# stijnherfst/Tyrant

Measured on AMD Instinct MI355X. Metric: Mrays/s at 1080p 8spp, higher is better.
Workload: dtype f32

## Files before the change

### tyrant_amd/csrc/hip/traverse.hpp

```cpp
#pragma once

#include <type_traits>

#include <hip/hip_runtime.h>

#include "vecmath.hpp"

namespace tyr {

constexpr uint32_t kRefLeaf = 0x80000000u;
constexpr uint32_t kRefDone = 0xFFFFFFFFu;
constexpr uint32_t kRefPop = 0xFFFFFFFEu;
constexpr int kStackSize = 64;
constexpr uint32_t kMaxLeafPrims = 31;
constexpr uint32_t kMaxPrimOffset = 1u << 26;
constexpr uint32_t kStagedNodes = 64;
constexpr uint32_t kQuadOrderShift = 25;
constexpr uint32_t kQuadIndexMask = (1u << kQuadOrderShift) - 1u;

struct DevScene {
	const float4* quads;
	uint32_t quadRootRef;
	uint32_t nQuads;
	uint32_t nStaged;
// ... 177 lines not shown
		lds = (lds_column_t)ldsColumn;
		spillRef = refs;
		spillT = ts;
	}
	__device__ __forceinline__ void reset() {
		n = 0;
		overflow = false;
	}
	__device__ __forceinline__ void lds_put(int d, uint32_t r, float t) {
		if constexpr (WITH_T)
			lds[d * kBlockThreads] = make_uint2(r, __float_as_uint(t));
		else
			lds[d * kBlockThreads] = r;
	}
	__device__ __forceinline__ void lds_get(int d, uint32_t& r, float& t) {
		if constexpr (WITH_T) {
			const uint2 e = lds[d * kBlockThreads];
			r = e.x;
			t = __uint_as_float(e.y);
		} else {
			r = lds[d * kBlockThreads];
			t = -__builtin_inff();
		}
	}
	__device__ __forceinline__ void push(uint32_t r, float t) {
		if (LDS_DEPTH > 0 && n < LDS_DEPTH) {
			lds_put(n, r, t);
			++n;
		} else if (n < kStackSize) {
			spillRef[n - LDS_DEPTH] = r;
			if (WITH_T)
				spillT[n - LDS_DEPTH] = t;
			++n;
		} else {
			overflow = true;
		}
	}
	__device__ __forceinline__ bool pop(uint32_t& r, float& t) {
		if (n == 0)
			return false;
		if (LDS_DEPTH > 0 && __builtin_amdgcn_ballot_w64(n > LDS_DEPTH) == 0ull) {
			--n;
			lds_get(n, r, t);
			return true;
		}
		--n;
		if (LDS_DEPTH > 0 && n < LDS_DEPTH) {
			lds_get(n, r, t);
		} else {
			r = spillRef[n - LDS_DEPTH];
			t = WITH_T ? spillT[n - LDS_DEPTH] : -__builtin_inff();
		}
		return true;
	}
	__device__ __forceinline__ void push3(unsigned long long ma, uint32_t ra, float ta, unsigned long long mb, uint32_t rb, float tb, unsigned long long mc, uint32_t rc, float tc) {
		if (LDS_DEPTH >= 3 && __builtin_amdgcn_ballot_w64(n > LDS_DEPTH - 3) == 0ull) {
			if (__builtin_amdgcn_inverse_ballot_w64(ma)) {
				lds_put(n, ra, ta);
				++n;
			}
			if (__builtin_amdgcn_inverse_ballot_w64(mb)) {
				lds_put(n, rb, tb);
				++n;
			}
			if (__builtin_amdgcn_inverse_ballot_w64(mc)) {
				lds_put(n, rc, tc);
				++n;
			}
			return;
		}
		if (__builtin_amdgcn_inverse_ballot_w64(ma))
			push(ra, ta);
		if (__builtin_amdgcn_inverse_ballot_w64(mb))
			push(rb, tb);
		if (__builtin_amdgcn_inverse_ballot_w64(mc))
			push(rc, tc);
	}
};

struct PairTest {
	uint32_t nearRef, farRef;
	float nearT, farT;
	bool nearHit, farHit;
	bool synthetic;
};

__device__ __forceinline__ PairTest test_pair(const float4* __restrict__ nodes, uint32_t idx, const RayConst& r, float dist) {
	const float4 qx = nodes[4 * idx + 0];
	const float4 qy = nodes[4 * idx + 1];
	const float4 qz = nodes[4 * idx + 2];
	const float4 qr = nodes[4 * idx + 3];
	const uint32_t leftRef = __float_as_uint(qr.x), rightRef = __float_as_uint(qr.y), axis = __float_as_uint(qr.z);
	float tL, tR;
	const bool hL = slab_test(r, r.nx ? qx.y : qx.x, r.nx ? qx.x : qx.y, r.ny ? qy.y : qy.x, r.ny ? qy.x : qy.y, r.nz ? qz.y : qz.x, r.nz ? qz.x : qz.y, dist, tL);
	const bool hR = slab_test(r, r.nx ? qx.w : qx.z, r.nx ? qx.z : qx.w, r.ny ? qy.w : qy.z, r.ny ? qy.z : qy.w, r.nz ? qz.w : qz.z, r.nz ? qz.z : qz.w, dist, tR);
	const bool rightFirst = (axis == 0) ? r.nx : (axis == 1) ? r.ny : (axis == 2) ? r.nz : false;
	PairTest p;
	p.nearRef = rightFirst ? rightRef : leftRef;
	p.farRef = rightFirst ? leftRef : rightRef;
	p.nearT = rightFirst ? tR : tL;
	p.farT = rightFirst ? tL : tR;
	p.nearHit = rightFirst ? hR : hL;
	p.farHit = rightFirst ? hL : hR;
	p.synthetic = (axis == 3);
	if (p.synthetic) {
		p.nearHit = true;
// ... 85 lines not shown
#if defined(__HIP_DEVICE_COMPILE__)
		typedef __attribute__((address_space(3))) const float4* lds_f4;
		const lds_f4 c = (lds_f4)staged + idx;
#else
		const float4* c = staged + idx;
#endif
		x01 = c[0 * STAGE_STRIDE], x23 = c[1 * STAGE_STRIDE], y01 = c[2 * STAGE_STRIDE], y23 = c[3 * STAGE_STRIDE];
		z01 = c[4 * STAGE_STRIDE], z23 = c[5 * STAGE_STRIDE], rf = c[6 * STAGE_STRIDE];
		__asm__ volatile("" : "+v"(rf.x));
	} else {
		x01 = q[0], x23 = q[1], y01 = q[2], y23 = q[3], z01 = q[4], z23 = q[5], rf = q[6];
	}
	const uint32_t r0 = __float_as_uint(rf.x), r1 = __float_as_uint(rf.y), r2 = __float_as_uint(rf.z), r3 = __float_as_uint(rf.w);
	float t0, t1, t2, t3;
	const lanemask H0 = slab_any<FAST>(r, x01.x, x01.y, y01.x, y01.y, z01.x, z01.y, dist, t0);
	const lanemask H1 = slab_any<FAST>(r, x01.z, x01.w, y01.z, y01.w, z01.z, z01.w, dist, t1);
	const lanemask H2 = slab_any<FAST>(r, x23.x, x23.y, y23.x, y23.y, z23.x, z23.y, dist, t2);
	const lanemask H3 = slab_any<FAST>(r, x23.z, x23.w, y23.z, y23.w, z23.z, z23.w, dist, t3);
	if (!ORDERED) {
		QuadHits o;
		o.ref[0] = r0, o.ref[1] = r1, o.ref[2] = r2, o.ref[3] = r3;
		o.t[0] = t0, o.t[1] = t1, o.t[2] = t2, o.t[3] = t3;
		o.hit[0] = H0, o.hit[1] = H1, o.hit[2] = H2, o.hit[3] = H3;
		return o;
	}
	const uint32_t signBits = (r.nx ? 1u : 0u) | (r.ny ? 2u : 0u) | (r.nz ? 4u : 0u);
	const uint32_t aT = meta & 3u, aL = (meta >> 2) & 3u, aR = (meta >> 4) & 3u;
	const bool bT = ((signBits >> aT) & 1u) != 0u;
	const bool bL = ((signBits >> aL) & 1u) != 0u;
	const bool bR = ((signBits >> aR) & 1u) != 0u;
	const lanemask BT = lanes_where(bT), BL = lanes_where(bL), BR = lanes_where(bR);
	const uint32_t lr0 = bL ? r1 : r0, lr1 = bL ? r0 : r1;
	const float lt0 = bL ? t1 : t0, lt1 = bL ? t0 : t1;
	const lanemask LH0 = mask_select(BL, H1, H0), LH1 = mask_select(BL, H0, H1);
	const uint32_t rr0 = bR ? r3 : r2, rr1 = bR ? r2 : r3;
	const float rt0 = bR ? t3 : t2, rt1 = bR ? t2 : t3;
	const lanemask RH0 = mask_select(BR, H3, H2), RH1 = mask_select(BR, H2, H3);
	QuadHits o;
	o.ref[0] = bT ? rr0 : lr0;
	o.ref[1] = bT ? rr1 : lr1;
	o.ref[2] = bT ? lr0 : rr0;
	o.ref[3] = bT ? lr1 : rr1;
	o.t[0] = bT ? rt0 : lt0;
	o.t[1] = bT ? rt1 : lt1;
	o.t[2] = bT ? lt0 : rt0;
	o.t[3] = bT ? lt1 : rt1;
	o.hit[0] = mask_select(BT, RH0, LH0);
	o.hit[1] = mask_select(BT, RH1, LH1);
	o.hit[2] = mask_select(BT, LH0, RH0);
	o.hit[3] = mask_select(BT, LH1, RH1);
	return o;
}

struct VisitCount {
	uint32_t nodes, tris;
};

template <bool COUNT, class Stack>
__device__ __forceinline__ bool bvh_closest(const DevScene& sc, const RayConst& r, float& dist, int& prim, Stack& st, VisitCount& vc) {
	bool hit = false;
	st.reset();
	uint32_t ref;
	{
		float t0;
		const bool ok = slab_test(r, r.nx ? sc.rootMax[0] : sc.rootMin[0], r.nx ? sc.rootMin[0] : sc.rootMax[0], r.ny ? sc.rootMax[1] : sc.rootMin[1], r.ny ? sc.rootMin[1] : sc.rootMax[1],
			r.nz ? sc.rootMax[2] : sc.rootMin[2], r.nz ? sc.rootMin[2] : sc.rootMax[2], dist, t0);
		if (COUNT)
			vc.nodes += 1;
		ref = ok ? sc.rootRef : kRefDone;
	}
	while (ref != kRefDone) {
		while ((int)ref >= 0) {
			const PairTest p = test_pair(sc.nodes, ref, r, dist);
			if (COUNT && !p.synthetic)
				vc.nodes += 2;
			if (p.nearHit) {
				if (p.farHit)
					st.push(p.farRef, p.farT);
				ref = p.nearRef;
			} else if (p.farHit) {
				ref = p.farRef;
			} else {
				ref = kRefDone;
				uint32_t pr;
				float pt;
				while (st.pop(pr, pt)) {
					if (pt < dist) {
						ref = pr;
						break;
					}
				}
			}
		}
		if (ref == kRefDone)
			break;
		const uint32_t off = ref & (kMaxPrimOffset - 1);
		const uint32_t cnt = ((ref >> 26) & 31u) + 1u;
		for (uint32_t i = 0; i < cnt; ++i) {
			const float t = triangle_test(sc.tris, off + i, r);
			if (COUNT)
				vc.tris += 1;
			if (t > kEpsilon && t < dist && ((dist - t) > kEpsilon)) {
				prim = (int)(off + i);
				dist = t;
				hit = true;
			}
// ... 88 lines not shown
```

### tyrant_amd/csrc/hip/traverse_flat.hip

```cpp
#include "device_common.hpp"
#include "scan_wave.hpp"

namespace tyr {

constexpr uint32_t kTraceBlockWide = 768;
#define TYR_FLAT_WAVES_PER_EU (STACK_LDS <= 8 ? 6 : STACK_LDS <= 12 ? 5 : STACK_LDS <= 16 ? 3 : 2)

__device__ __forceinline__ bool ref_is_leaf(uint32_t ref) { return (ref & kRefLeaf) && ref < kRefPop; }
__device__ __forceinline__ bool ref_is_traversing(uint32_t ref) { return ((int)ref >= 0) || ref == kRefPop; }
__device__ __forceinline__ unsigned long long lanes_traversing(uint32_t ref) { return __builtin_amdgcn_ballot_w64((int)ref >= 0) | __builtin_amdgcn_ballot_w64(ref == kRefPop); }
__device__ __forceinline__ unsigned long long lanes_at_leaf(uint32_t ref) { return __builtin_amdgcn_ballot_w64((ref & kRefLeaf) != 0u) & __builtin_amdgcn_ballot_w64(ref < kRefPop); }

#ifdef TYR_QUAD_STATS
constexpr bool kLoopStats = true;
#else
constexpr bool kLoopStats = false;
#endif
#if defined(TYR_QUAD_STATS) || defined(TYR_LAUNCH_ANATOMY)
constexpr bool kAnatomy = true;
#else
constexpr bool kAnatomy = false;
#endif
#define TYR_DBG(i)                                                     \
	if (COUNT || kLoopStats) {                                         \
// ... 344 lines not shown
			TriData tri = triangle_load(sc.tris, off);
			for (uint32_t i = 0; i < cnt && !found; ++i) {
				const TriData cur = tri;
				if (i + 1 < cnt)
					tri = triangle_load(sc.tris, off + i + 1);
				const float t = triangle_test(cur, r);
				vc.tris += 1;
				found = (t > kEpsilon && ((closest - t) > kEpsilon));
			}
			if (found) {
				occluded = true;
				ref = kRefDone;
			} else {
				ref = kRefPop;
			}
		}
		if (live && ref == kRefDone) {
			if (!occluded) {
				pendIdx = index;
				visible += 1;
			}
			overflow = overflow || st.overflow;
			live = false;
		}
	}
	flush_visible();
	if (overflow)
		atomicOr(&P.k->device_error, kErrStackOverflow);
	if (kGuardPasses && passes > kMaxPasses)
		atomicOr(&P.k->device_error, kErrNoProgress);
	wave_add_u64(&P.k->n_shadow_visible, visible);
	wave_add_u64(&P.k->nodes_connect, vc.nodes);
	wave_add_u64(&P.k->tris_connect, vc.tris);
	wave_add_u64(&P.k->rays_in_tree_connect, inTree);
}

__device__ __forceinline__ void wave_lds_order() {
	__builtin_amdgcn_fence(__ATOMIC_RELEASE, "wavefront");
	__builtin_amdgcn_wave_barrier();
	__builtin_amdgcn_fence(__ATOMIC_ACQUIRE, "wavefront");
}
template <int CTRL>
__device__ __forceinline__ uint32_t quad_perm_u(uint32_t v) { return (uint32_t)__builtin_amdgcn_mov_dpp((int)v, CTRL, 0xf, 0xf, true); }
__device__ __forceinline__ uint32_t quad_or(uint32_t v) {
	v |= quad_perm_u<0xB1>(v);
	v |= quad_perm_u<0x4E>(v);
	return v;
}
template <int K>
__device__ __forceinline__ float quad_bcast_f(float v) { return __uint_as_float(quad_perm_u<K * 0x55>(__float_as_uint(v))); }
#define TYR_GLOBAL __attribute__((address_space(1)))
typedef float v2f_t __attribute__((ext_vector_type(2)));
typedef float v4f_t __attribute__((ext_vector_type(4)));
__device__ __forceinline__ float2 gload_f2(const float* p) {
	const v2f_t v = *(const TYR_GLOBAL v2f_t*)p;
	return make_float2(v.x, v.y);
}
__device__ __forceinline__ float4 gload_f4(const float4* p) {
	const v4f_t v = *(const TYR_GLOBAL v4f_t*)p;
	return make_float4(v.x, v.y, v.z, v.w);
}
__device__ __forceinline__ uint32_t gload_u(const float* p) { return *(const TYR_GLOBAL uint32_t*)p; }
__device__ __forceinline__ TriData triangle_gload(const float4* tris, uint32_t prim) {
	TriData d;
	d.a = gload_f4(tris + 3 * prim + 0);
	d.b = gload_f4(tris + 3 * prim + 1);
	d.c = make_float4(__uint_as_float(gload_u(reinterpret_cast<const float*>(tris + 3 * prim + 2))), 0.0f, 0.0f, 0.0f);
	return d;
}
constexpr uint32_t kWideRays = 16;
constexpr int kWideStackEntries = 4 * 12;

#ifdef TYR_LAUNCH_ANATOMY
#define TYR_WIDE_STEPS_PARAM , uint32_t& wideSteps
#define TYR_WIDE_STEPS_ARG , wideSteps
#else
#define TYR_WIDE_STEPS_PARAM
#define TYR_WIDE_STEPS_ARG
#endif
struct WideState {
	float rox, roy, roz, rdx, rdy, rdz, rix, riy, riz, dist;
	uint32_t ref, slot, flags;
	int prim, n;
};
template <int STACK_LDS>
__device__ __attribute__((noinline, cold)) uint32_t wide_drain(const float4* __restrict__ quads, const float4* __restrict__ tris, const float4* __restrict__ shadowColor, const float4* __restrict__ shadowDyzCdIx,
                                                         float2* __restrict__ workHit, float4* __restrict__ blit, typename LdsStack<STACK_LDS, true>::entry_t* smem_, WideState w, uint32_t passes TYR_WIDE_STEPS_PARAM) {
	const uint32_t lane = lane_id();
	const unsigned long long below = (1ull << lane) - 1ull;
	float rox = w.rox, roy = w.roy, roz = w.roz, rdx = w.rdx, rdy = w.rdy, rdz = w.rdz, rix = w.rix, riy = w.riy, riz = w.riz, dist = w.dist;
	uint32_t ref = w.ref, slot = w.slot;
	int prim = w.prim;
	bool regular = (w.flags & 1u) != 0u, hitTri = (w.flags & 2u) != 0u, isShadow = (w.flags & 4u) != 0u, occluded = (w.flags & 8u) != 0u;
	const bool live = (w.flags & 16u) != 0u;
	uint32_t visible = 0;
	struct { int n; } st = { w.n };
	const uint32_t sub = lane & 3u, grp = lane >> 2;
	const unsigned long long lm = __ballot(live);
	const uint32_t nl = (uint32_t)__popcll(lm);
	const uint32_t told = (uint32_t)__builtin_amdgcn_ds_permute(live ? (int)(__popcll(lm & below) << 2) : 63 * 4, (int)lane);
	bool gActive = grp < nl;
	const uint32_t asked = (uint32_t)__builtin_amdgcn_ds_bpermute((int)(grp << 2), (int)told);
	const uint32_t srcLane = gActive ? asked : lane;
	const int pull = (int)(srcLane << 2);
	auto pull_f = [&](float v) { return __uint_as_float((uint32_t)__builtin_amdgcn_ds_bpermute(pull, (int)__float_as_uint(v))); };
	auto pull_u = [&](uint32_t v) { return (uint32_t)__builtin_amdgcn_ds_bpermute(pull, (int)v); };
	rox = pull_f(rox), roy = pull_f(roy), roz = pull_f(roz);
	rdx = pull_f(rdx), rdy = pull_f(rdy), rdz = pull_f(rdz);
	rix = pull_f(rix), riy = pull_f(riy), riz = pull_f(riz);
	dist = pull_f(dist);
	ref = pull_u(ref);
	slot = pull_u(slot);
	prim = (int)pull_u((uint32_t)prim);
	const uint32_t fl = pull_u((regular ? 1u : 0u) | (hitTri ? 2u : 0u) | (isShadow ? 4u : 0u) | (occluded ? 8u : 0u));
	regular = (fl & 1u) != 0u, hitTri = (fl & 2u) != 0u, isShadow = (fl & 4u) != 0u, occluded = (fl & 8u) != 0u;
	int n = (int)pull_u((uint32_t)st.n);
	typedef typename LdsStack<STACK_LDS, true>::entry_t entry_t;
	entry_t* const column0 = smem_ + (threadIdx.x >> 8) * (STACK_LDS * kBlock) + (threadIdx.x & 255u & ~63u);
	entry_t moved[STACK_LDS / 4];
#pragma unroll
	for (int row = 0; row < STACK_LDS / 4; ++row) {
		const int e = 4 * row + (int)sub;
		moved[row] = (gActive && e < n) ? column0[e * kBlock + srcLane] : entry_t{};
	}
	wave_lds_order();
#pragma unroll
	for (int row = 0; row < STACK_LDS / 4; ++row)
		if (gActive && 4 * row + (int)sub < n)
			column0[row * kBlock + lane] = moved[row];
	wave_lds_order();
	entry_t* const gstack = column0 + (lane & ~3u);
	const RayConst r = { mk3(rox, roy, roz), mk3(rdx, rdy, rdz), mk3(rix, riy, riz), rix < 0, riy < 0, riz < 0 };
	const uint32_t signBits = (r.nx ? 1u : 0u) | (r.ny ? 2u : 0u) | (r.nz ? 4u : 0u);
	bool wideOverflow = false;
	const bool allRegular = __ballot(gActive && !regular) == 0ull;
	while (__ballot(gActive) != 0ull) {
		if (kGuardPasses && ++passes > kMaxPasses)
			break;
#ifdef TYR_LAUNCH_ANATOMY
		wideSteps += 1;
#endif
		{
			const bool popping = gActive && ref == kRefPop;
			const bool has = n > 0;
			const int top = has ? n - 1 : 0;
			const entry_t e = gstack[(top >> 2) * kBlock + (top & 3)];
			const uint32_t popped = !has ? kRefDone : (__uint_as_float(e.y) < dist ? e.x : kRefPop);
			ref = popping ? popped : ref;
			n = (popping && has) ? n - 1 : n;
		}
		const bool atNode = gActive && (int)ref >= 0;
		if (__ballot(atNode) != 0ull) {
			const uint32_t idx = atNode ? (ref & kQuadIndexMask) : 0u, meta = ref >> kQuadOrderShift;
			const float* qf = reinterpret_cast<const float*>(quads + 8 * idx);
			const uint32_t at = (sub >> 1) * 4u + (sub & 1u) * 2u;
			const float2 bx = gload_f2(qf + at);
			const float2 by = gload_f2(qf + 8 + at);
			const float2 bz = gload_f2(qf + 16 + at);
			const uint32_t cref = gload_u(qf + 24 + sub);
			float t;
			bool h;
			if (allRegular)
				h = slab_fast(r, bx.x, bx.y, by.x, by.y, bz.x, bz.y, dist, t);
			else
				h = slab_test(r, r.nx ? bx.y : bx.x, r.nx ? bx.x : bx.y, r.ny ? by.y : by.x, r.ny ? by.x : by.y, r.nz ? bz.y : bz.x, r.nz ? bz.x : bz.y, dist, t);
			h = h && atNode;
			const uint32_t aT = meta & 3u, aL = (meta >> 2) & 3u, aR = (meta >> 4) & 3u;
			const uint32_t bT = (signBits >> aT) & 1u, bG = (signBits >> ((sub >> 1) ? aR : aL)) & 1u;
			const uint32_t rank = 2u * ((sub >> 1) ^ bT) + ((sub & 1u) ^ bG);
			const uint32_t hr = quad_or(h ? (1u << rank) : 0u);
			const uint32_t first = (uint32_t)__ffs((int)(hr | 16u)) - 1u;
			const int e = n + (int)__popc(hr >> (rank + 1u));
			if (h && rank != first && e < kWideStackEntries)
				gstack[(e >> 2) * kBlock + (e & 3)] = make_uint2(cref, __float_as_uint(t));
			int n2 = n + (int)__popc(hr) - (hr != 0u ? 1 : 0);
			wideOverflow = wideOverflow || (atNode && n2 > kWideStackEntries);
			n2 = n2 > kWideStackEntries ? kWideStackEntries : n2;
			const uint32_t nearest = quad_or((h && rank == first) ? cref : 0u);
			ref = atNode ? (hr == 0u ? kRefPop : nearest) : ref;
			n = atNode ? n2 : n;
		}
		const bool atLeaf = gActive && ref_is_leaf(ref);
		if (__ballot(atLeaf) != 0ull) {
			const uint32_t off = ref & (kMaxPrimOffset - 1);
			const uint32_t cnt = atLeaf ? ((ref >> 26) & 31u) + 1u : 0u;
			bool found = false;
			for (uint32_t base = 0; __ballot(base < cnt) != 0ull; base += 4u) {
				const uint32_t i = base + sub;
				const bool mine = i < cnt;
				const TriData td = triangle_gload(tris, mine ? off + i : 0u);
				float tm = triangle_test_select(td, r);
				tm = mine ? tm : 0.0f;
				const float t0 = quad_bcast_f<0>(tm), t1 = quad_bcast_f<1>(tm), t2 = quad_bcast_f<2>(tm), t3 = quad_bcast_f<3>(tm);
				const float tk[4] = { t0, t1, t2, t3 };
#pragma unroll
				for (uint32_t k = 0; k < 4u; ++k) {
					const float t = tk[k];
					const bool in = (base + k < cnt) && t > kEpsilon && ((dist - t) > kEpsilon);
					found = found || (in && isShadow);
					const bool closer = in && !isShadow && t < dist;
					prim = closer ? (int)(off + base + k) : prim;
					hitTri = hitTri || closer;
					dist = closer ? t : dist;
				}
			}
			occluded = occluded || found;
			ref = atLeaf ? (found ? kRefDone : kRefPop) : ref;
		}
		if (gActive && ref == kRefDone) {
			if (sub == 0u) {
				if (isShadow) {
					if (!occluded) {
						const float4 c = shadowColor[slot];
						accumulate_pixel(blit, __float_as_int(shadowDyzCdIx[slot].w), mk3(c.x, c.y, c.z), 0);
						visible += 1;
					}
				} else {
					finish_extend_ray(workHit, slot, hitTri, dist, prim);
				}
			}
			gActive = false;
		}
	}
	return visible | (wideOverflow ? 0x80000000u : 0u) | (kGuardPasses && passes > kMaxPasses ? 0x40000000u : 0u);
}

template <int STACK_LDS, uint32_t kTraceBlock>
#define TYR_TRACE_VIEW(name) const FrameParams& name = kernarg_view<FrameParams>();
__global__ void __launch_bounds__(kTraceBlock, (kTraceBlock == kTraceBlockWide ? 6 : TYR_FLAT_WAVES_PER_EU)) k_trace_flat(const FrameParams P) {
	constexpr bool COUNT = false;
	__shared__ typename LdsStack<STACK_LDS, true>::entry_t smem_[STACK_LDS * kTraceBlock];
	uint32_t spillRef_[kStackSize - STACK_LDS];
	float spillT_[kStackSize - STACK_LDS];
	LdsStack<STACK_LDS, true> st;
	st.bind(smem_ + (threadIdx.x >> 8) * (STACK_LDS * kBlock) + (threadIdx.x & 255u), spillRef_, spillT_);
	st.reset();
	__shared__ float4 stagedNodes[7 * kStagedNodes];
	__shared__ uint32_t blockNext;
	const uint32_t nStaged = P.scene.nStaged;
	for (uint32_t i = threadIdx.x; i < 7 * nStaged; i += kTraceBlock) {
		const uint32_t v = i / nStaged, n = i - v * nStaged;
		stagedNodes[v * kStagedNodes + n] = P.scene.quads[8 * n + v];
	}
	const uint32_t lane = lane_id();
	const unsigned long long below = (1ull << lane) - 1ull;
	[[maybe_unused]] uint32_t tripsFeed = 0;
	const uint32_t nExt = P.traceShadow == 2u ? 0u : queue_extent(P.segWork);
	const uint32_t nItems = nExt + (P.traceShadow != 0u ? queue_extent(P.kcPrev->seg) : 0u);
	const DevScene& sc = P.scene;
	float rox = 0.f, roy = 0.f, roz = 0.f, rdx = 0.f, rdy = 0.f, rdz = 0.f, rix = 0.f, riy = 0.f, riz = 0.f;
	bool regular = true, allRegular = true;
	float dist = 0.0f;
	uint32_t ref = kRefDone, slot = 0;
	int prim = 0;
	bool hitTri = false, live = false, overflow = false;
	bool isShadow = false, occluded = false;
	uint32_t visible = 0;
	uint32_t dbg[16] = {};
	uint32_t steps = 0;
	[[maybe_unused]] unsigned long long tExhausted = 0ull, tWide = 0ull;
	[[maybe_unused]] uint32_t liveAtExhaustion = 0, liveAtWide = 0, tripsAfter = 0, passesAfter = 0, wideSteps = 0;
	const unsigned long long tStart = kAnatomy ? __builtin_amdgcn_s_memrealtime() : 0ull;
	constexpr uint32_t kNoPending = 0xffffffffu;
	uint32_t pendIdx = kNoPending;
	auto flush_visible = [&]() {
		TYR_TRACE_VIEW(P)
		float4 c = make_float4(0.f, 0.f, 0.f, 0.f);
		int px = 0;
		if (pendIdx != kNoPending) {
			c = P.shadowPrev.color[pendIdx];
			px = __float_as_int(P.shadowPrev.dyz_cd_ix[pendIdx].w);
		}
		accumulate_pixels_wave(P.blit, px, mk3(c.x, c.y, c.z), 0);
		pendIdx = kNoPending;
// ... 66 lines not shown
				TYR_DBG(6)
				float4 a;
				float by, bz, bound;
				bool blocked = false;
				if (s < nExt) {
					a = P.work.o_dx[s];
					const float2 b = P.work.dyz[s];
					const float2 h = P.work.hit[s];
					by = b.x, bz = b.y, bound = h.x;
					slot = s;
					isShadow = false;
				} else {
					const uint32_t idx = s - nExt;
					a = P.shadowPrev.o_dx[idx];
					const float4 b = P.shadowPrev.dyz_cd_ix[idx];
					blocked = reinterpret_cast<const float*>(&P.shadowPrev.color[idx])[3] != 0.0f;
					by = b.x, bz = b.y, bound = b.z;
					slot = idx;
					isShadow = true;
				}
				const RayConst nr = make_ray(mk3(a.x, a.y, a.z), mk3(a.w, by, bz));
				rox = nr.o.x, roy = nr.o.y, roz = nr.o.z, rdx = nr.d.x, rdy = nr.d.y, rdz = nr.d.z, rix = nr.inv.x, riy = nr.inv.y, riz = nr.inv.z;
				regular = ray_is_regular(nr);
				dist = bound;
				hitTri = false;
				occluded = blocked;
				st.reset();
				ref = blocked ? kRefDone : root_ref(sc, nr, dist);
				if (ref != kRefDone)
					ref = sc.quadRootRef;
				live = (ref != kRefDone) || (isShadow && !blocked);
			}
			if (!exhausted && (uint32_t)__popcll(__ballot(live && ref != kRefDone)) < P.minTraversing)
				if (__ballot(live && ref == kRefDone) == 0ull)
					continue;
		}
		{
			const uint32_t nLiveNow = (uint32_t)__popcll(__ballot(live));
			if (exhausted && nLiveNow <= wideLimit && __ballot(live && st.n > STACK_LDS) == 0ull) {
				wide = nLiveNow != 0u;
				if (kAnatomy) {
					tWide = __builtin_amdgcn_s_memrealtime();
					liveAtWide = nLiveNow;
				}
				break;
			}
			if (kAnatomy && exhausted)
				passesAfter += 1;
			if (nLiveNow == 0u)
				continue;
		}
		allRegular = (__ballot(live && !regular) == 0ull);
		const RayConst r = { mk3(rox, roy, roz), mk3(rdx, rdy, rdz), mk3(rix, riy, riz), rix < 0, riy < 0, riz < 0 };
		for (;;) {
			const uint32_t nTrav = __popcll(lanes_traversing(ref));
			if (nTrav == 0)
				break;
			if (nTrav < P.minTraversing) {
				const bool anyLeaf = lanes_at_leaf(ref) != 0ull;
				const bool canRefill = !exhausted && (uint32_t)__popcll(__ballot(!live || ref == kRefDone)) >= P.refillMinIdle;
				if (anyLeaf || canRefill)
					break;
			}
			if (kAnatomy && exhausted)
				tripsAfter += 1;
			if (kAnatomy && !exhausted)
				tripsFeed += 1;
			if (ref == kRefPop) {
				TYR_DBG(2)
				uint32_t pr;
				float pt;
				if (st.pop(pr, pt)) {
					if (pt < dist)
						ref = pr;
				} else {
					ref = kRefDone;
				}
			}
			if ((int)ref >= 0) {
				TYR_DBG(0)
				if (kLoopStats)
					steps += 1;
				const QuadHits q = allRegular ? test_quad<true, true, true>(sc.quads, ref, r, dist, stagedNodes, nStaged) : test_quad<false, true, true>(sc.quads, ref, r, dist, stagedNodes, nStaged);
				const lanemask any01 = q.hit[0] | q.hit[1], any012 = any01 | q.hit[2];
				st.push3(q.hit[3] & any012, q.ref[3], q.t[3], q.hit[2] & any01, q.ref[2], q.t[2], q.hit[1] & q.hit[0], q.ref[1], q.t[1]);
				ref = lane_in(q.hit[0]) ? q.ref[0] : lane_in(q.hit[1]) ? q.ref[1] : lane_in(q.hit[2]) ? q.ref[2] : lane_in(q.hit[3]) ? q.ref[3] : kRefPop;
			}
		}
		{
			const bool atLeaf = ref_is_leaf(ref);
			const unsigned long long B0 = __ballot(atLeaf);
			if (B0 != 0ull) {
				const uint32_t off = ref & (kMaxPrimOffset - 1);
				const uint32_t cnt = atLeaf ? ((ref >> 26) & 31u) + 1u : 0u;
				const unsigned long long B1 = __ballot(cnt > 1u), B2 = __ballot(cnt > 2u), B3 = __ballot(cnt > 3u);
				const uint32_t n0 = (uint32_t)__popcll(B0), n1 = (uint32_t)__popcll(B1), n2 = (uint32_t)__popcll(B2), n3 = (uint32_t)__popcll(B3);
				if (__ballot(cnt > 4u) == 0ull && n0 + n1 + n2 + n3 <= 63u) {
					const uint32_t base1 = n0, base2 = n0 + n1, base3 = n0 + n1 + n2;
					const uint32_t s0 = (uint32_t)__popcll(B0 & below), s1 = base1 + (uint32_t)__popcll(B1 & below), s2 = base2 + (uint32_t)__popcll(B2 & below), s3 = base3 + (uint32_t)__popcll(B3 & below);
					const uint32_t me = lane + 1u;
					uint32_t told = (uint32_t)__builtin_amdgcn_ds_permute((int)((cnt > 0u ? s0 : 63u) << 2), (int)(cnt > 0u ? me : 0u));
					if (n1)
						told |= (uint32_t)__builtin_amdgcn_ds_permute((int)((cnt > 1u ? s1 : 63u) << 2), (int)(cnt > 1u ? (me | (1u << 8)) : 0u));
					if (n2)
						told |= (uint32_t)__builtin_amdgcn_ds_permute((int)((cnt > 2u ? s2 : 63u) << 2), (int)(cnt > 2u ? (me | (2u << 8)) : 0u));
					if (n3)
						told |= (uint32_t)__builtin_amdgcn_ds_permute((int)((cnt > 3u ? s3 : 63u) << 2), (int)(cnt > 3u ? (me | (3u << 8)) : 0u));
					const bool item = lane < n0 + n1 + n2 + n3;
					const int from = (int)((item ? (told & 0xffu) - 1u : lane) << 2);
					auto pull = [&](float v) { return __uint_as_float((uint32_t)__builtin_amdgcn_ds_bpermute(from, (int)__float_as_uint(v))); };
					const uint32_t offO = (uint32_t)__builtin_amdgcn_ds_bpermute(from, (int)off);
					RayConst ro;
					ro.o = mk3(pull(rox), pull(roy), pull(roz));
					ro.d = mk3(pull(rdx), pull(rdy), pull(rdz));
					if ((COUNT || kLoopStats) && item) {
						TYR_DBG(4)
					}
					float tm = triangle_test_select(triangle_load(sc.tris, item ? offO + (told >> 8) : 0u), ro);
					tm = item ? tm : 0.0f;
					const float t0 = __uint_as_float((uint32_t)__builtin_amdgcn_ds_bpermute((int)(s0 << 2), (int)__float_as_uint(tm)));
					const float t1 = n1 ? __uint_as_float((uint32_t)__builtin_amdgcn_ds_bpermute((int)(s1 << 2), (int)__float_as_uint(tm))) : 0.0f;
					const float t2 = n2 ? __uint_as_float((uint32_t)__builtin_amdgcn_ds_bpermute((int)(s2 << 2), (int)__float_as_uint(tm))) : 0.0f;
					const float t3 = n3 ? __uint_as_float((uint32_t)__builtin_amdgcn_ds_bpermute((int)(s3 << 2), (int)__float_as_uint(tm))) : 0.0f;
					const float tk[4] = { t0, t1, t2, t3 };
					bool found = false;
#pragma unroll
					for (uint32_t i = 0; i < 4u; ++i) {
						const float t = tk[i];
						const bool in = i < cnt && !found && t > kEpsilon && ((dist - t) > kEpsilon);
						const bool closer = in && !isShadow && t < dist;
						found = found || (in && isShadow);
						prim = closer ? (int)(off + i) : prim;
						hitTri = hitTri || closer;
						dist = closer ? t : dist;
					}
					if (atLeaf) {
						occluded = occluded || found;
						ref = found ? kRefDone : kRefPop;
					}
				}
			}
		}
		if (ref_is_leaf(ref)) {
			const uint32_t off = ref & (kMaxPrimOffset - 1);
			const uint32_t cnt = ((ref >> 26) & 31u) + 1u;
			bool found = false;
			TriData tri = triangle_load(sc.tris, off);
			for (uint32_t i = 0; i < cnt && !found; ++i) {
				TYR_DBG(4)
				const TriData cur = tri;
				if (i + 1 < cnt)
					tri = triangle_load(sc.tris, off + i + 1);
				const float t = triangle_test(cur, r);
				if (isShadow) {
					found = (t > kEpsilon && ((dist - t) > kEpsilon));
				} else if (t > kEpsilon && t < dist && ((dist - t) > kEpsilon)) {
					prim = (int)(off + i);
					dist = t;
					hitTri = true;
				}
			}
			occluded = occluded || found;
			ref = found ? kRefDone : kRefPop;
		}
		if (live && ref == kRefDone) {
			if (isShadow) {
				if (!occluded) {
					pendIdx = slot;
					visible += 1;
				}
			} else {
				finish_extend_ray(P.work.hit, slot, hitTri, dist, prim);
			}
			overflow = overflow || st.overflow;
			live = false;
			if (kLoopStats) {
				atomicMax(&P.k->debug[12], (unsigned long long)steps);
				if (steps > 64)
					atomicAdd(&P.k->debug[9], 1ull);
				if (steps > 128)
					atomicAdd(&P.k->debug[10], 1ull);
				if (steps > 256)
					atomicAdd(&P.k->debug[11], 1ull);
				steps = 0;
			}
		}
	}
	flush_visible();
	TYR_TRACE_VIEW(PE)
	if (wide) {
		WideState w;
		w.rox = rox, w.roy = roy, w.roz = roz, w.rdx = rdx, w.rdy = rdy, w.rdz = rdz, w.rix = rix, w.riy = riy, w.riz = riz, w.dist = dist;
		w.ref = ref, w.slot = slot, w.prim = prim, w.n = st.n;
		w.flags = (regular ? 1u : 0u) | (hitTri ? 2u : 0u) | (isShadow ? 4u : 0u) | (occluded ? 8u : 0u) | (live ? 16u : 0u);
		const uint32_t res = wide_drain<STACK_LDS>(PE.scene.quads, PE.scene.tris, PE.shadowPrev.color, PE.shadowPrev.dyz_cd_ix, PE.work.hit, PE.blit, smem_, w, passes TYR_WIDE_STEPS_ARG);
		visible += res & 0x3fffffffu;
		overflow = overflow || (res & 0x80000000u) != 0u;
		if (res & 0x40000000u)
			passes = kMaxPasses + 1;
	}
	if (overflow)
		atomicOr(&PE.k->device_error, kErrStackOverflow);
	if (kGuardPasses && passes > kMaxPasses)
		atomicOr(&PE.k->device_error, kErrNoProgress);
	wave_add_u64(&PE.k->n_shadow_visible, visible);
	if (kLoopStats) {
		for (int i = 0; i < 9; ++i)
			wave_add_u64(&PE.k->debug[i], dbg[i]);
	}
	if (kAnatomy && lane == 0) {
		const unsigned long long tEnd = __builtin_amdgcn_s_memrealtime();
		atomicMax(&P.k->debug[13], ~tStart);
		atomicMax(&P.k->debug[14], ~(tExhausted ? tExhausted : tEnd));
		atomicMax(&P.k->debug[15], tEnd);
		const uint32_t w = blockIdx.x * (kTraceBlock / 64) + (threadIdx.x >> 6);
		if (w < P.N)
			P.next.hit[w] = make_float2((float)((tExhausted ? tExhausted : tEnd) - tStart) * 0.01f, (float)(tEnd - tStart) * 0.01f + (float)liveAtExhaustion * 0.0f);
		if (w < 8192u && 32768u < P.N) {
			P.next.hit[8192u + w] = make_float2(tWide ? (float)(tWide - tStart) * 0.01f : 0.0f, (float)(liveAtExhaustion + 256u * liveAtWide));
			P.next.hit[16384u + w] = make_float2((float)tripsAfter, (float)wideSteps);
			P.next.hit[24576u + w] = make_float2((float)passesAfter, (float)tripsFeed);
		}
	}
}

#undef TYR_DBG
#undef TYR_TRACE_VIEW


#define TYR_TRACE_STACK 12
void launch_trace(const FrameParams& P, uint32_t maxLive, uint32_t nSurvivors, uint32_t maxShadowPrev, const Tuning& t, int numCUs, LaunchCache& lc, hipStream_t stream) {
	launch_trace_prepasses(P, nSurvivors, maxShadowPrev, stream, maxLive);
	launch_trace_kernel(P, maxLive + maxShadowPrev, t, numCUs, lc, stream);
}
void launch_trace_kernel(const FrameParams& P, uint32_t items, const Tuning& t, int numCUs, LaunchCache& lc, hipStream_t stream) {
	if (t.wideBlockMinItems >= 0 && items >= (uint32_t)t.wideBlockMinItems)
		hipLaunchKernelGGL((k_trace_flat<TYR_TRACE_STACK, kTraceBlockWide>), dim3(persistent_blocks(k_trace_flat<TYR_TRACE_STACK, kTraceBlockWide>, items, t, numCUs, lc.perCU[kLcTrace][1], kTraceBlockWide)), dim3(kTraceBlockWide), 0, stream, P);
	else
		hipLaunchKernelGGL((k_trace_flat<TYR_TRACE_STACK, (uint32_t)kBlock>), dim3(persistent_blocks(k_trace_flat<TYR_TRACE_STACK, (uint32_t)kBlock>, items, t, numCUs, lc.perCU[kLcTrace][0])), dim3(kBlock), 0, stream, P);
}
void launch_trace_prepasses(const FrameParams& P, uint32_t nSurvivors, uint32_t maxShadowPrev, hipStream_t stream, uint32_t maxLive) {
	FrameParams Pc = P;
	Pc.kc = P.kcPrev;
	Pc.shadow = P.shadowPrev;
	if (P.prevFolded) {
		if (!P.prologueDone)
			launch_pad_holes(Pc, P.traceShadow != 2u, maxShadowPrev != 0, stream, P.traceShadow == 2u);
		return;
// ... 42 lines not shown
```

Measured before the change: 8086.

## Use rank-based push/pop in traversal and slim wide-drain call interface

The main traversal loop replaces the sorted-order quad hit handling with rank bitmasks computed from the node's split-axis metadata. It also uses a branchless pop_select and a push_ranked that writes stack entries at popcount-derived slots. The cold wide_drain function now takes scalar arguments plus the kernarg pointer instead of a struct and six pointers, uses wave-uniform lanemasks for state, and uses byte-offset global loads. The aim is to cut VALU work, divergent branches and the register and call overhead in the hot loop, at the cost of more complex indexing logic.

```diff
diff --git a/tyrant_amd/csrc/hip/traverse.hpp b/tyrant_amd/csrc/hip/traverse.hpp
--- a/tyrant_amd/csrc/hip/traverse.hpp
+++ b/tyrant_amd/csrc/hip/traverse.hpp
@@ -253,6 +253,58 @@
 			t = WITH_T ? spillT[n - LDS_DEPTH] : -__builtin_inff();
 		}
 		return true;
+	}
+	__device__ __forceinline__ void pop_select(bool popping, uint32_t& ref, float bound) {
+		if (LDS_DEPTH > 0 && __builtin_amdgcn_ballot_w64(popping && n > LDS_DEPTH) == 0ull) {
+			const bool take = popping && n > 0;
+			uint32_t r;
+			float t;
+			lds_get(take ? n - 1 : 0, r, t);
+			ref = popping ? (n == 0 ? kRefDone : (t < bound ? r : kRefPop)) : ref;
+			n = take ? n - 1 : n;
+			return;
+		}
+		if (popping) {
+			if (n == 0) {
+				ref = kRefDone;
+			} else {
+				--n;
+				uint32_t r;
+				float t;
+				if (LDS_DEPTH > 0 && n < LDS_DEPTH) {
+					lds_get(n, r, t);
+				} else {
+					r = spillRef[n - LDS_DEPTH];
+					t = WITH_T ? spillT[n - LDS_DEPTH] : -__builtin_inff();
+				}
+				if (t < bound)
+					ref = r;
+			}
+		}
+	}
+	__device__ __forceinline__ void push_ranked(const uint32_t* ref, const float* t, const unsigned long long* hit, const uint32_t* rank, uint32_t hr, uint32_t first) {
+		if (LDS_DEPTH >= 3 && __builtin_amdgcn_ballot_w64(n > LDS_DEPTH - 3) == 0ull) {
+			const uint32_t after = hr >> 1;
+#pragma unroll
+			for (int s = 0; s < 4; ++s)
+				if (__builtin_amdgcn_inverse_ballot_w64(hit[s]) && rank[s] != first)
+					lds_put(n + (int)__popc(after >> rank[s]), ref[s], t[s]);
+			n += (int)__popc(hr) - (hr != 0u ? 1 : 0);
+			return;
+		}
+		uint32_t oref[4];
+		float ot[4];
+#pragma unroll
+		for (uint32_t k = 1; k < 4; ++k) {
+			oref[k] = rank[0] == k ? ref[0] : rank[1] == k ? ref[1] : rank[2] == k ? ref[2] : ref[3];
+			ot[k] = rank[0] == k ? t[0] : rank[1] == k ? t[1] : rank[2] == k ? t[2] : t[3];
+		}
+		if ((hr & 8u) && (hr & 7u))
+			push(oref[3], ot[3]);
+		if ((hr & 4u) && (hr & 3u))
+			push(oref[2], ot[2]);
+		if ((hr & 2u) && (hr & 1u))
+			push(oref[1], ot[1]);
 	}
 	__device__ __forceinline__ void push3(unsigned long long ma, uint32_t ra, float ta, unsigned long long mb, uint32_t rb, float tb, unsigned long long mc, uint32_t rc, float tc) {
 		if (LDS_DEPTH >= 3 && __builtin_amdgcn_ballot_w64(n > LDS_DEPTH - 3) == 0ull) {
@@ -444,6 +496,17 @@
 	return o;
 }
 
+__device__ __forceinline__ void quad_ranks(uint32_t ref, uint32_t signBits, uint32_t* rank) {
+	const uint32_t bT = __builtin_amdgcn_ubfe(signBits, __builtin_amdgcn_ubfe(ref, kQuadOrderShift, 2u), 1u);
+	const uint32_t bL = __builtin_amdgcn_ubfe(signBits, __builtin_amdgcn_ubfe(ref, kQuadOrderShift + 2u, 2u), 1u);
+	const uint32_t bR = __builtin_amdgcn_ubfe(signBits, __builtin_amdgcn_ubfe(ref, kQuadOrderShift + 4u, 2u), 1u);
+	const uint32_t xL = (bT << 1) | bL, xR = (bT << 1) | bR;
+	rank[0] = xL;
+	rank[1] = xL ^ 1u;
+	rank[2] = xR ^ 2u;
+	rank[3] = xR ^ 3u;
+}
+
 struct VisitCount {
 	uint32_t nodes, tris;
 };
diff --git a/tyrant_amd/csrc/hip/traverse_flat.hip b/tyrant_amd/csrc/hip/traverse_flat.hip
--- a/tyrant_amd/csrc/hip/traverse_flat.hip
+++ b/tyrant_amd/csrc/hip/traverse_flat.hip
@@ -420,20 +420,22 @@
 #define TYR_GLOBAL __attribute__((address_space(1)))
 typedef float v2f_t __attribute__((ext_vector_type(2)));
 typedef float v4f_t __attribute__((ext_vector_type(4)));
-__device__ __forceinline__ float2 gload_f2(const float* p) {
-	const v2f_t v = *(const TYR_GLOBAL v2f_t*)p;
+__device__ __forceinline__ const TYR_GLOBAL char* gbytes(const void* base, uint32_t byteOffset) { return (const TYR_GLOBAL char*)base + byteOffset; }
+__device__ __forceinline__ float2 gload_f2(const void* base, uint32_t byteOffset) {
+	const v2f_t v = *(const TYR_GLOBAL v2f_t*)gbytes(base, byteOffset);
 	return make_float2(v.x, v.y);
 }
-__device__ __forceinline__ float4 gload_f4(const float4* p) {
-	const v4f_t v = *(const TYR_GLOBAL v4f_t*)p;
+__device__ __forceinline__ float4 gload_f4(const void* base, uint32_t byteOffset) {
+	const v4f_t v = *(const TYR_GLOBAL v4f_t*)gbytes(base, byteOffset);
 	return make_float4(v.x, v.y, v.z, v.w);
 }
-__device__ __forceinline__ uint32_t gload_u(const float* p) { return *(const TYR_GLOBAL uint32_t*)p; }
+__device__ __forceinline__ uint32_t gload_u(const void* base, uint32_t byteOffset) { return *(const TYR_GLOBAL uint32_t*)gbytes(base, byteOffset); }
 __device__ __forceinline__ TriData triangle_gload(const float4* tris, uint32_t prim) {
+	const uint32_t at = prim * 48u;
 	TriData d;
-	d.a = gload_f4(tris + 3 * prim + 0);
-	d.b = gload_f4(tris + 3 * prim + 1);
-	d.c = make_float4(__uint_as_float(gload_u(reinterpret_cast<const float*>(tris + 3 * prim + 2))), 0.0f, 0.0f, 0.0f);
+	d.a = gload_f4(tris, at);
+	d.b = gload_f4(tris, at + 16u);
+	d.c = make_float4(__uint_as_float(gload_u(tris, at + 32u)), 0.0f, 0.0f, 0.0f);
 	return d;
 }
 constexpr uint32_t kWideRays = 16;
@@ -446,23 +448,16 @@
 #define TYR_WIDE_STEPS_PARAM
 #define TYR_WIDE_STEPS_ARG
 #endif
-struct WideState {
-	float rox, roy, roz, rdx, rdy, rdz, rix, riy, riz, dist;
-	uint32_t ref, slot, flags;
-	int prim, n;
-};
+constexpr uint32_t kWideRegular = 1u, kWideHitTri = 2u, kWideShadow = 4u, kWideOccluded = 8u, kWideLive = 16u;
 template <int STACK_LDS>
-__device__ __attribute__((noinline, cold)) uint32_t wide_drain(const float4* __restrict__ quads, const float4* __restrict__ tris, const float4* __restrict__ shadowColor, const float4* __restrict__ shadowDyzCdIx,
-                                                         float2* __restrict__ workHit, float4* __restrict__ blit, typename LdsStack<STACK_LDS, true>::entry_t* smem_, WideState w, uint32_t passes TYR_WIDE_STEPS_PARAM) {
+__device__ __attribute__((noinline, cold)) uint32_t wide_drain(unsigned long long kernarg, typename LdsStack<STACK_LDS, true>::lds_column_t smem_, float rox, float roy, float roz, float rdx, float rdy, float rdz, float rix, float riy, float riz, float dist,
+                                                         uint32_t ref, uint32_t slot, int prim, uint32_t flags, int n, uint32_t passes TYR_WIDE_STEPS_PARAM) {
+	const unsigned long long ka = (unsigned long long)(uint32_t)__builtin_amdgcn_readfirstlane((int)(uint32_t)kernarg) | ((unsigned long long)(uint32_t)__builtin_amdgcn_readfirstlane((int)(uint32_t)(kernarg >> 32)) << 32);
+	const FrameParams& P = *(const FrameParams*)(const __attribute__((address_space(4))) FrameParams*)ka;
 	const uint32_t lane = lane_id();
 	const unsigned long long below = (1ull << lane) - 1ull;
-	float rox = w.rox, roy = w.roy, roz = w.roz, rdx = w.rdx, rdy = w.rdy, rdz = w.rdz, rix = w.rix, riy = w.riy, riz = w.riz, dist = w.dist;
-	uint32_t ref = w.ref, slot = w.slot;
-	int prim = w.prim;
-	bool regular = (w.flags & 1u) != 0u, hitTri = (w.flags & 2u) != 0u, isShadow = (w.flags & 4u) != 0u, occluded = (w.flags & 8u) != 0u;
-	const bool live = (w.flags & 16u) != 0u;
+	const bool live = (flags & kWideLive) != 0u;
 	uint32_t visible = 0;
-	struct { int n; } st = { w.n };
 	const uint32_t sub = lane & 3u, grp = lane >> 2;
 	const unsigned long long lm = __ballot(live);
 	const uint32_t nl = (uint32_t)__popcll(lm);
@@ -480,11 +475,13 @@
 	ref = pull_u(ref);
 	slot = pull_u(slot);
 	prim = (int)pull_u((uint32_t)prim);
-	const uint32_t fl = pull_u((regular ? 1u : 0u) | (hitTri ? 2u : 0u) | (isShadow ? 4u : 0u) | (occluded ? 8u : 0u));
-	regular = (fl & 1u) != 0u, hitTri = (fl & 2u) != 0u, isShadow = (fl & 4u) != 0u, occluded = (fl & 8u) != 0u;
-	int n = (int)pull_u((uint32_t)st.n);
+	const uint32_t fl = pull_u(flags);
+	const bool regular = (fl & kWideRegular) != 0u, isShadow = (fl & kWideShadow) != 0u;
+	bool hitTri = (fl & kWideHitTri) != 0u, occluded = (fl & kWideOccluded) != 0u;
+	n = (int)pull_u((uint32_t)n);
 	typedef typename LdsStack<STACK_LDS, true>::entry_t entry_t;
-	entry_t* const column0 = smem_ + (threadIdx.x >> 8) * (STACK_LDS * kBlock) + (threadIdx.x & 255u & ~63u);
+	typedef typename LdsStack<STACK_LDS, true>::lds_column_t lds_ptr_t;
+	const lds_ptr_t column0 = smem_ + (threadIdx.x >> 8) * (STACK_LDS * kBlock) + (threadIdx.x & 255u & ~63u);
 	entry_t moved[STACK_LDS / 4];
 #pragma unroll
 	for (int row = 0; row < STACK_LDS / 4; ++row) {
@@ -497,97 +494,104 @@
 		if (gActive && 4 * row + (int)sub < n)
 			column0[row * kBlock + lane] = moved[row];
 	wave_lds_order();
-	entry_t* const gstack = column0 + (lane & ~3u);
+	const lds_ptr_t gstack = column0 + (lane & ~3u);
+	auto entry_at = [&](int e) { return gstack + (((uint32_t)e >> 2) * kBlock + ((uint32_t)e & 3u)); };
 	const RayConst r = { mk3(rox, roy, roz), mk3(rdx, rdy, rdz), mk3(rix, riy, riz), rix < 0, riy < 0, riz < 0 };
 	const uint32_t signBits = (r.nx ? 1u : 0u) | (r.ny ? 2u : 0u) | (r.nz ? 4u : 0u);
+	const uint32_t boxAt = (sub >> 1) * 16u + (sub & 1u) * 8u, refAt = 96u + 4u * sub, groupBits = kQuadOrderShift + 2u + 2u * (sub >> 1);
+	const float4* const quads = P.scene.quads;
+	const float4* const tris = P.scene.tris;
+	const lanemask shadowM = __ballot(isShadow);
+	lanemask act = __ballot(gActive), hitM = __ballot(hitTri), occM = __ballot(occluded);
 	bool wideOverflow = false;
-	const bool allRegular = __ballot(gActive && !regular) == 0ull;
-	while (__ballot(gActive) != 0ull) {
+	const bool allRegular = (act & ~__ballot(regular)) == 0ull;
+	while (act != 0ull) {
 		if (kGuardPasses && ++passes > kMaxPasses)
 			break;
 #ifdef TYR_LAUNCH_ANATOMY
 		wideSteps += 1;
 #endif
 		{
-			const bool popping = gActive && ref == kRefPop;
+			const bool popping = lane_in(act & lanes_where(ref == kRefPop));
 			const bool has = n > 0;
-			const int top = has ? n - 1 : 0;
-			const entry_t e = gstack[(top >> 2) * kBlock + (top & 3)];
+			const entry_t e = *entry_at(has ? n - 1 : 0);
 			const uint32_t popped = !has ? kRefDone : (__uint_as_float(e.y) < dist ? e.x : kRefPop);
 			ref = popping ? popped : ref;
 			n = (popping && has) ? n - 1 : n;
 		}
-		const bool atNode = gActive && (int)ref >= 0;
-		if (__ballot(atNode) != 0ull) {
-			const uint32_t idx = atNode ? (ref & kQuadIndexMask) : 0u, meta = ref >> kQuadOrderShift;
-			const float* qf = reinterpret_cast<const float*>(quads + 8 * idx);
-			const uint32_t at = (sub >> 1) * 4u + (sub & 1u) * 2u;
-			const float2 bx = gload_f2(qf + at);
-			const float2 by = gload_f2(qf + 8 + at);
-			const float2 bz = gload_f2(qf + 16 + at);
-			const uint32_t cref = gload_u(qf + 24 + sub);
+		const lanemask nodeM = act & lanes_where((int)ref >= 0);
+		if (nodeM != 0ull) {
+			const bool atNode = lane_in(nodeM);
+			const uint32_t node = (atNode ? (ref & kQuadIndexMask) : 0u) * 128u;
+			const float2 bx = gload_f2(quads, node + boxAt);
+			const float2 by = gload_f2(quads, node + boxAt + 32u);
+			const float2 bz = gload_f2(quads, node + boxAt + 64u);
+			const uint32_t cref = gload_u(quads, node + refAt);
 			float t;
-			bool h;
+			lanemask H;
 			if (allRegular)
-				h = slab_fast(r, bx.x, bx.y, by.x, by.y, bz.x, bz.y, dist, t);
+				H = slab_fast_mask(r, bx.x, bx.y, by.x, by.y, bz.x, bz.y, dist, t);
 			else
-				h = slab_test(r, r.nx ? bx.y : bx.x, r.nx ? bx.x : bx.y, r.ny ? by.y : by.x, r.ny ? by.x : by.y, r.nz ? bz.y : bz.x, r.nz ? bz.x : bz.y, dist, t);
-			h = h && atNode;
-			const uint32_t aT = meta & 3u, aL = (meta >> 2) & 3u, aR = (meta >> 4) & 3u;
-			const uint32_t bT = (signBits >> aT) & 1u, bG = (signBits >> ((sub >> 1) ? aR : aL)) & 1u;
-			const uint32_t rank = 2u * ((sub >> 1) ^ bT) + ((sub & 1u) ^ bG);
+				H = lanes_where(slab_test(r, r.nx ? bx.y : bx.x, r.nx ? bx.x : bx.y, r.ny ? by.y : by.x, r.ny ? by.x : by.y, r.nz ? bz.y : bz.x, r.nz ? bz.x : bz.y, dist, t));
+			const bool h = lane_in(H & nodeM);
+			const uint32_t bT = __builtin_amdgcn_ubfe(signBits, __builtin_amdgcn_ubfe(ref, kQuadOrderShift, 2u), 1u);
+			const uint32_t bG = __builtin_amdgcn_ubfe(signBits, __builtin_amdgcn_ubfe(ref, groupBits, 2u), 1u);
+			const uint32_t rank = sub ^ ((bT << 1) | bG);
 			const uint32_t hr = quad_or(h ? (1u << rank) : 0u);
-			const uint32_t first = (uint32_t)__ffs((int)(hr | 16u)) - 1u;
-			const int e = n + (int)__popc(hr >> (rank + 1u));
-			if (h && rank != first && e < kWideStackEntries)
-				gstack[(e >> 2) * kBlock + (e & 3)] = make_uint2(cref, __float_as_uint(t));
-			int n2 = n + (int)__popc(hr) - (hr != 0u ? 1 : 0);
-			wideOverflow = wideOverflow || (atNode && n2 > kWideStackEntries);
-			n2 = n2 > kWideStackEntries ? kWideStackEntries : n2;
-			const uint32_t nearest = quad_or((h && rank == first) ? cref : 0u);
-			ref = atNode ? (hr == 0u ? kRefPop : nearest) : ref;
-			n = atNode ? n2 : n;
-		}
-		const bool atLeaf = gActive && ref_is_leaf(ref);
-		if (__ballot(atLeaf) != 0ull) {
+			const bool nearest = h && (hr & (0u - hr)) == (1u << rank);
+			const int e = n + (int)__popc(hr >> rank >> 1);
+			if (h && !nearest && e < kWideStackEntries)
+				*entry_at(e) = make_uint2(cref, __float_as_uint(t));
+			const int n2 = n + (int)__popc(hr) - (hr != 0u ? 1 : 0);
+			wideOverflow = wideOverflow || (nodeM & lanes_where(n2 > kWideStackEntries)) != 0ull;
+			const uint32_t next = quad_or(nearest ? cref : 0u);
+			ref = atNode ? (hr == 0u ? kRefPop : next) : ref;
+			n = atNode ? (n2 > kWideStackEntries ? kWideStackEntries : n2) : n;
+		}
+		const lanemask leafM = act & lanes_at_leaf(ref);
+		if (leafM != 0ull) {
+			const bool atLeaf = lane_in(leafM);
 			const uint32_t off = ref & (kMaxPrimOffset - 1);
 			const uint32_t cnt = atLeaf ? ((ref >> 26) & 31u) + 1u : 0u;
-			bool found = false;
+			lanemask inM = 0ull;
 			for (uint32_t base = 0; __ballot(base < cnt) != 0ull; base += 4u) {
 				const uint32_t i = base + sub;
 				const bool mine = i < cnt;
 				const TriData td = triangle_gload(tris, mine ? off + i : 0u);
 				float tm = triangle_test_select(td, r);
 				tm = mine ? tm : 0.0f;
-				const float t0 = quad_bcast_f<0>(tm), t1 = quad_bcast_f<1>(tm), t2 = quad_bcast_f<2>(tm), t3 = quad_bcast_f<3>(tm);
-				const float tk[4] = { t0, t1, t2, t3 };
+				const float tk[4] = { quad_bcast_f<0>(tm), quad_bcast_f<1>(tm), quad_bcast_f<2>(tm), quad_bcast_f<3>(tm) };
+				uint32_t took = 4u;
 #pragma unroll
 				for (uint32_t k = 0; k < 4u; ++k) {
 					const float t = tk[k];
-					const bool in = (base + k < cnt) && t > kEpsilon && ((dist - t) > kEpsilon);
-					found = found || (in && isShadow);
-					const bool closer = in && !isShadow && t < dist;
-					prim = closer ? (int)(off + base + k) : prim;
-					hitTri = hitTri || closer;
-					dist = closer ? t : dist;
-				}
-			}
-			occluded = occluded || found;
-			ref = atLeaf ? (found ? kRefDone : kRefPop) : ref;
-		}
-		if (gActive && ref == kRefDone) {
-			if (sub == 0u) {
+					const lanemask in = lanes_where(t > kEpsilon) & lanes_where((dist - t) > kEpsilon);
+					const lanemask closer = in & ~shadowM;
+					inM |= in;
+					hitM |= closer;
+					dist = lane_in(closer) ? t : dist;
+					took = lane_in(closer) ? k : took;
+				}
+				prim = took != 4u ? (int)(off + base + took) : prim;
+			}
+			const lanemask foundM = inM & shadowM & leafM;
+			occM |= foundM;
+			ref = atLeaf ? (lane_in(foundM) ? kRefDone : kRefPop) : ref;
+		}
+		const lanemask finM = act & lanes_where(ref == kRefDone);
+		if (finM != 0ull) {
+			if (lane_in(finM) && sub == 0u) {
 				if (isShadow) {
-					if (!occluded) {
-						const float4 c = shadowColor[slot];
-						accumulate_pixel(blit, __float_as_int(shadowDyzCdIx[slot].w), mk3(c.x, c.y, c.z), 0);
+					if (!lane_in(occM)) {
+						const v4f_t c = ((const TYR_GLOBAL v4f_t*)P.shadowPrev.color)[slot];
+						accumulate_pixel(P.blit, __float_as_int(((const TYR_GLOBAL v4f_t*)P.shadowPrev.dyz_cd_ix)[slot].w), mk3(c.x, c.y, c.z), 0);
 						visible += 1;
 					}
-				} else {
-					finish_extend_ray(workHit, slot, hitTri, dist, prim);
-				}
-			}
-			gActive = false;
+				} else if (lane_in(hitM)) {
+					((TYR_GLOBAL v2f_t*)P.work.hit)[slot] = v2f_t{ dist, __uint_as_float((uint32_t)prim) };
+				}
+			}
+			act &= ~finM;
 		}
 	}
 	return visible | (wideOverflow ? 0x80000000u : 0u) | (kGuardPasses && passes > kMaxPasses ? 0x40000000u : 0u);
@@ -760,6 +764,7 @@
 		}
 		allRegular = (__ballot(live && !regular) == 0ull);
 		const RayConst r = { mk3(rox, roy, roz), mk3(rdx, rdy, rdz), mk3(rix, riy, riz), rix < 0, riy < 0, riz < 0 };
+		const uint32_t signBits = (r.nx ? 1u : 0u) | (r.ny ? 2u : 0u) | (r.nz ? 4u : 0u);
 		for (;;) {
 			const uint32_t nTrav = __popcll(lanes_traversing(ref));
 			if (nTrav == 0)
@@ -774,25 +779,21 @@
 				tripsAfter += 1;
 			if (kAnatomy && !exhausted)
 				tripsFeed += 1;
-			if (ref == kRefPop) {
+			if (kLoopStats && ref == kRefPop) {
 				TYR_DBG(2)
-				uint32_t pr;
-				float pt;
-				if (st.pop(pr, pt)) {
-					if (pt < dist)
-						ref = pr;
-				} else {
-					ref = kRefDone;
-				}
-			}
+			}
+			st.pop_select(ref == kRefPop, ref, dist);
 			if ((int)ref >= 0) {
 				TYR_DBG(0)
 				if (kLoopStats)
 					steps += 1;
-				const QuadHits q = allRegular ? test_quad<true, true, true>(sc.quads, ref, r, dist, stagedNodes, nStaged) : test_quad<false, true, true>(sc.quads, ref, r, dist, stagedNodes, nStaged);
-				const lanemask any01 = q.hit[0] | q.hit[1], any012 = any01 | q.hit[2];
-				st.push3(q.hit[3] & any012, q.ref[3], q.t[3], q.hit[2] & any01, q.ref[2], q.t[2], q.hit[1] & q.hit[0], q.ref[1], q.t[1]);
-				ref = lane_in(q.hit[0]) ? q.ref[0] : lane_in(q.hit[1]) ? q.ref[1] : lane_in(q.hit[2]) ? q.ref[2] : lane_in(q.hit[3]) ? q.ref[3] : kRefPop;
+				const QuadHits q = allRegular ? test_quad<true, false, true>(sc.quads, ref, r, dist, stagedNodes, nStaged) : test_quad<false, false, true>(sc.quads, ref, r, dist, stagedNodes, nStaged);
+				uint32_t rank[4];
+				quad_ranks(ref, signBits, rank);
+				const uint32_t hr = (lane_in(q.hit[0]) ? 1u << rank[0] : 0u) | (lane_in(q.hit[1]) ? 1u << rank[1] : 0u) | (lane_in(q.hit[2]) ? 1u << rank[2] : 0u) | (lane_in(q.hit[3]) ? 1u << rank[3] : 0u);
+				const uint32_t first = (uint32_t)__ffs((int)hr) - 1u;
+				st.push_ranked(q.ref, q.t, q.hit, rank, hr, first);
+				ref = rank[0] == first ? q.ref[0] : rank[1] == first ? q.ref[1] : rank[2] == first ? q.ref[2] : rank[3] == first ? q.ref[3] : kRefPop;
 			}
 		}
 		{
@@ -897,11 +898,8 @@
 	flush_visible();
 	TYR_TRACE_VIEW(PE)
 	if (wide) {
-		WideState w;
-		w.rox = rox, w.roy = roy, w.roz = roz, w.rdx = rdx, w.rdy = rdy, w.rdz = rdz, w.rix = rix, w.riy = riy, w.riz = riz, w.dist = dist;
-		w.ref = ref, w.slot = slot, w.prim = prim, w.n = st.n;
-		w.flags = (regular ? 1u : 0u) | (hitTri ? 2u : 0u) | (isShadow ? 4u : 0u) | (occluded ? 8u : 0u) | (live ? 16u : 0u);
-		const uint32_t res = wide_drain<STACK_LDS>(PE.scene.quads, PE.scene.tris, PE.shadowPrev.color, PE.shadowPrev.dyz_cd_ix, PE.work.hit, PE.blit, smem_, w, passes TYR_WIDE_STEPS_ARG);
+		const uint32_t flags = (regular ? kWideRegular : 0u) | (hitTri ? kWideHitTri : 0u) | (isShadow ? kWideShadow : 0u) | (occluded ? kWideOccluded : 0u) | (live ? kWideLive : 0u);
+		const uint32_t res = wide_drain<STACK_LDS>((unsigned long long)__builtin_amdgcn_kernarg_segment_ptr(), (typename LdsStack<STACK_LDS, true>::lds_column_t)smem_, rox, roy, roz, rdx, rdy, rdz, rix, riy, riz, dist, ref, slot, prim, flags, st.n, passes TYR_WIDE_STEPS_ARG);
 		visible += res & 0x3fffffffu;
 		overflow = overflow || (res & 0x80000000u) != 0u;
 		if (res & 0x40000000u)
```

After: 8298, median of 6. 1.03x the previous value.
